# yanqinJiang/Animate3D

Measured on AMD Instinct MI355X. Metric: UNet denoise-steps/sec, 4view×16frame×512² MV-VDM @1/2/4/8 GPU, higher is better.
Workload: dtype bf16; 1 GPU; BASELINE config 2: 4 views x 16 frames x 512^2 px (64x64 latent), CFG-doubled batch V=8 videos, one MVUNetMotionModel.forward per step, SD1.5 MV-VDM UNet 1.53 B params, seeded synthetic weights; parallelism=single GPU

## Files before the change

### animate3d_amd/csrc/gemm_conv.hip

```cpp
#include "gemm_common.h"

namespace {

constexpr int BM = 128, BN = 128;
template <int BKT> struct TileCfg {
  static constexpr int LROW = BKT + 8;
  static constexpr int TILE_ELEMS = 128 * LROW;
  static constexpr int STAGE_BYTES = 2 * 2 * TILE_ELEMS * 2;
  static constexpr int EPI_BYTES = 4 * 32 * 68 * 4;
  static constexpr int SMEM_BYTES = STAGE_BYTES > EPI_BYTES ? STAGE_BYTES : EPI_BYTES;
  static constexpr int CPR = BKT / 8;
  static constexpr int RPT = 256 / CPR;
  static constexpr int NPASS = 128 / RPT;
};



template <int CONV, int EPI, int BKT, bool RES>
__global__ __launch_bounds__(256, (BKT == 64 ? 2 : 3)) void gemm_kernel(const GemmParams p) {
  using TC = TileCfg<BKT>;
  constexpr int LROW = TC::LROW, TILE_ELEMS = TC::TILE_ELEMS, NPASS = TC::NPASS, RPT = TC::RPT, BK = BKT;
  extern __shared__ __attribute__((aligned(16))) uint16_t smem[];
  const int tid = threadIdx.x;
  const int lane = tid & 63, wid = tid >> 6;
// ... 459 lines not shown
  p.X = (const uint16_t*)X; p.ldx = ldx; p.W = (const uint16_t*)W; p.ldw = ldw;
  p.bias = bias; p.rowbias = (const uint16_t*)rowbias; p.rb_div = rowbias ? rb_div : 1;
  p.R = (const uint16_t*)R; p.ldr = ldr; p.Y = (uint16_t*)Y; p.ldy = ldy;
  p.M = M; p.N = N; p.K = K; p.alpha = alpha; p.beta = beta;
  p.vec16 = (ldy % 8 == 0) && aligned16(Y) && (!R || (ldr % 8 == 0 && aligned16(R))) && (!rowbias || (N % 8 == 0 && aligned16(rowbias)));
  if (ws_needed) { *ws_needed = splitk_ws_bytes<0>(p, flags); return 0; }
  if (ws && ws_bytes > 0 && aligned16(ws)) { p.ws = (float*)ws; p.ws_bytes = ws_bytes; }
  return launch<0>((hipStream_t)stream, p, flags);
}

extern "C" int A3D_FN(a3d_gemm)(a3d_stream_t stream, const void* X, int64_t ldx, const void* W, int64_t ldw,
                             const float* bias, const void* rowbias, int64_t rb_div, const void* R, int64_t ldr,
                             void* Y, int64_t ldy, int64_t M, int64_t N, int64_t K, float alpha, float beta, int flags) {
  return gemm_entry(stream, X, ldx, W, ldw, bias, rowbias, rb_div, R, ldr, Y, ldy, M, N, K, alpha, beta, flags, nullptr, 0, nullptr);
}

extern "C" int A3D_FN(a3d_gemm_ws)(a3d_stream_t stream, const void* X, int64_t ldx, const void* W, int64_t ldw,
                                const float* bias, const void* rowbias, int64_t rb_div, const void* R, int64_t ldr,
                                void* Y, int64_t ldy, int64_t M, int64_t N, int64_t K, float alpha, float beta, int flags,
                                void* ws, int64_t ws_bytes, int64_t* ws_needed) {
  return gemm_entry(stream, X, ldx, W, ldw, bias, rowbias, rb_div, R, ldr, Y, ldy, M, N, K, alpha, beta, flags, ws, ws_bytes, ws_needed);
}

extern "C" int A3D_FN(a3d_gemm2)(a3d_stream_t stream, const void* X, int64_t ldx, const void* X2, int64_t ldx2, int64_t K1,
                              const void* W, int64_t ldw, const float* bias, void* Y, int64_t ldy, int64_t M, int64_t N, int64_t K, int flags) {
  if (!X || !X2 || !W || !Y || M <= 0 || N <= 0 || K <= 0 || K1 <= 0 || K1 >= K) return A3D_EINVAL;
  if (K % 64 != 0 || K1 % 64 != 0 || N % 8 != 0) return A3D_EINVAL;
  if (ldx % 8 != 0 || ldx2 % 8 != 0 || ldw % 8 != 0 || ldy % 8 != 0) return A3D_EINVAL;
  if (!aligned16(X) || !aligned16(X2) || !aligned16(W) || !aligned16(Y)) return A3D_EINVAL;
  if (bias && (reinterpret_cast<uintptr_t>(bias) & 15u)) return A3D_EINVAL;
  if (flags & ~(A3D_GEMM_RESERVED_CUS_MASK | A3D_GEMM_KERNEL_MASK)) return A3D_EINVAL;
  if (ldx2 % 64 != 0 || (uint64_t)ldx2 * 16u >= (1ull << 31)) return A3D_EUNSUPPORTED;
  GemmParams p{};
  p.X = (const uint16_t*)X; p.ldx = ldx; p.X2 = (const uint16_t*)X2; p.ldx2 = ldx2; p.K1 = K1;
  p.W = (const uint16_t*)W; p.ldw = ldw; p.bias = bias; p.rb_div = 1; p.Y = (uint16_t*)Y; p.ldy = ldy;
  p.M = M; p.N = N; p.K = K; p.alpha = 1.f; p.beta = 0.f; p.vec16 = 1;
  const int rc = try_launch_persist<0, EPI_LINEAR>((hipStream_t)stream, p, flags);
  return rc == -1000 ? A3D_EUNSUPPORTED : rc;
}

extern "C" int A3D_FN(a3d_gemm_f32out)(a3d_stream_t stream, const void* X, int64_t ldx, const void* W, int64_t ldw,
                                    const float* bias, float* Y, int64_t ldy, int64_t M, int64_t N, int64_t K, float alpha) {
  if (!X || !W || !Y || M <= 0 || N <= 0 || K <= 0) return A3D_EINVAL;
  if (K % 64 != 0 || N % 8 != 0 || ldx % 8 != 0 || ldw % 8 != 0 || ldy % 4 != 0) return A3D_EINVAL;
  if (!aligned16(X) || !aligned16(W) || !aligned16(Y)) return A3D_EINVAL;
  if (bias && (reinterpret_cast<uintptr_t>(bias) & 15u)) return A3D_EINVAL;
  GemmParams p{};
  p.X = (const uint16_t*)X; p.ldx = ldx; p.W = (const uint16_t*)W; p.ldw = ldw;
  p.bias = bias; p.rb_div = 1; p.Y = (uint16_t*)Y; p.ldy = ldy;
  p.M = M; p.N = N; p.K = K; p.alpha = alpha; p.beta = 0.f; p.vec16 = 1; p.out_f32 = 1;
  return launch<0>((hipStream_t)stream, p, 0);
}

static int conv_entry(a3d_stream_t stream, const void* X, const void* Wp, const float* bias,
                      const void* rowbias, int64_t rb_div, const void* R, void* Y,
                      int B, int H, int W, int Cin, int Cout, int stride, int up2x, int flags,
                      void* ws, int64_t ws_bytes, int64_t* ws_needed) {
  if (!X || !Wp || !Y || B <= 0 || H <= 0 || W <= 0) return A3D_EINVAL;
  if (Cin % 64 != 0 || Cout % 4 != 0 || (stride != 1 && stride != 2)) return A3D_EINVAL;
  if (up2x < 0 || up2x > 7 || (up2x > 1 && !(up2x & 1)) || (up2x && stride != 1)) return A3D_EINVAL;
  if (!aligned16(X) || !aligned16(Wp) || (reinterpret_cast<uintptr_t>(Y) & 7u)) return A3D_EINVAL;
// ... 43 lines not shown
```

### animate3d_amd/csrc/gemm_pp.hip

```cpp
#include "gemm_common.h"

namespace {

constexpr int PBM = 256;
template <int NB> struct PPCfg {
  static constexpr int BN = NB * 64;
  static constexpr int XBYTES = PBM * 128;
  static constexpr int WBYTES = BN * 128;
  static constexpr int EPI_BYTES = 8 * 32 * 68 * 4;
  static constexpr int STAGE = (XBYTES + WBYTES) > EPI_BYTES ? (XBYTES + WBYTES) : EPI_BYTES;
  static constexpr int BIAS_OFF = 2 * STAGE;
  static constexpr int BIAS_STRIDE = 2048;
  static constexpr int SMEM = 2 * STAGE + 2 * BIAS_STRIDE;
};

#ifndef A3D_PP_GM
#define A3D_PP_GM 8
#endif
constexpr int PP_GM = A3D_PP_GM;
A3D_DEV void pp_tile_coords(int64_t t, int64_t tiles_m, int64_t tiles_n, int64_t& tile_m, int64_t& tile_n) {
  const int64_t gsz = PP_GM * tiles_n;
  const int64_t blk = t / gsz;
  const int64_t first = blk * PP_GM;
  const int64_t gm = tiles_m - first < PP_GM ? tiles_m - first : PP_GM;
// ... 372 lines not shown
  static uint64_t attr_done = 0;
  if (int rc = a3d_once_per_device(attr_done, [] {
        return (int)hipFuncSetAttribute(reinterpret_cast<const void*>(&gemm_pp_kernel<CONV, EPI, NB, RES, SPLIT, TWO, DIRECT>),
                                        hipFuncAttributeMaxDynamicSharedMemorySize, PC::SMEM); })) return rc;
  const int64_t ntiles = p.tiles_m * p.tiles_n * (SPLIT ? p.ksplit : 1);
  const unsigned grid = (unsigned)(ntiles < cus ? ntiles : cus);
  gemm_pp_kernel<CONV, EPI, NB, RES, SPLIT, TWO, DIRECT><<<dim3(grid), dim3(512), PC::SMEM, stream>>>(p);
  if (int rc = a3d_launch_status()) return rc;
  if constexpr (SPLIT) {
    splitk_reduce_kernel<NB><<<dim3((unsigned)(p.tiles_m * p.tiles_n), NB), dim3(512), 0, stream>>>(p);
    return a3d_launch_status();
  }
  return 0;
}

template <int CONV>
int launch_pp_conv(int epi, int nb, hipStream_t stream, const GemmParams& p, int cus) {
  if (epi == EPI_GEGLU) {
    if constexpr (CONV == 0) { if (nb == 4) return launch_pp<0, EPI_GEGLU, 4, false>(stream, p, cus); }
    return A3D_EUNSUPPORTED;
  }
  if constexpr (CONV == 0) {
    if (p.X2 != nullptr) {
      if (p.R || p.ksplit > 1) return A3D_EUNSUPPORTED;
      if (nb == 5) return launch_pp<0, EPI_LINEAR, 5, false, false, true>(stream, p, cus);
      if (nb == 4) return launch_pp<0, EPI_LINEAR, 4, false, false, true>(stream, p, cus);
      return A3D_EUNSUPPORTED;
    }
  }
  if (p.ksplit > 1) {
    if (nb == 5) return launch_pp<CONV, EPI_LINEAR, 5, false, true>(stream, p, cus);
    if (nb == 4) return launch_pp<CONV, EPI_LINEAR, 4, false, true>(stream, p, cus);
    return A3D_EUNSUPPORTED;
  }
  if constexpr (CONV == 0) {
    if (p.direct) {
      if (nb == 5) return p.R ? launch_pp<0, EPI_LINEAR, 5, true, false, false, true>(stream, p, cus) : launch_pp<0, EPI_LINEAR, 5, false, false, false, true>(stream, p, cus);
      if (nb == 4) return p.R ? launch_pp<0, EPI_LINEAR, 4, true, false, false, true>(stream, p, cus) : launch_pp<0, EPI_LINEAR, 4, false, false, false, true>(stream, p, cus);
      return A3D_EUNSUPPORTED;
    }
  }
  if (nb == 5) return p.R ? launch_pp<CONV, EPI_LINEAR, 5, true>(stream, p, cus) : launch_pp<CONV, EPI_LINEAR, 5, false>(stream, p, cus);
  if (nb == 4) return p.R ? launch_pp<CONV, EPI_LINEAR, 4, true>(stream, p, cus) : launch_pp<CONV, EPI_LINEAR, 4, false>(stream, p, cus);
  return A3D_EUNSUPPORTED;
}

}

int A3D_FN(a3d_launch_gemm_pp)(int conv, int epi, int nb, hipStream_t stream, const GemmParams& p, int cus) {
// ... 5 lines not shown
```

### animate3d_amd/hip_ops.py

```python
from __future__ import annotations

import ctypes
import os
from dataclasses import dataclass
from typing import Optional

import torch

_LIB_PATH = os.path.join(os.path.dirname(os.path.abspath(__file__)), "lib", "libanimate3d_hip.so")
_lib = None

c_i64, c_int, c_f32, c_vp = ctypes.c_int64, ctypes.c_int, ctypes.c_float, ctypes.c_void_p


class _RowMapC(ctypes.Structure):
    _fields_ = [("gdiv", c_i64), ("ga", c_i64), ("gb", c_i64), ("seg_len", c_i64), ("seg_stride", c_i64), ("ld", c_i64)]


@dataclass(frozen=True)
class RowMap:
    gdiv: int
    ga: int
    gb: int
    seg_len: int
# ... 2 lines not shown
    def c(self, ld: int) -> _RowMapC:
        return _RowMapC(self.gdiv, self.ga, self.gb, self.seg_len, self.seg_stride, ld)


def rowmap_rows(m: RowMap, groups: int, step: int, length: int, device="cpu") -> torch.Tensor:
    g = torch.arange(0, groups, step, device=device).view(-1, 1)
    s = torch.arange(length, device=device).view(1, -1)
    return ((g // m.gdiv) * m.ga + (g % m.gdiv) * m.gb + (s // m.seg_len) * m.seg_stride + s % m.seg_len).reshape(-1)


def rowmap_covers(m: RowMap, groups: int, step: int, length: int, rows: int, device="cpu") -> bool:
    if (groups + step - 1) // step * length != rows:
        return False
    idx = rowmap_rows(m, groups, step, length, device)
    return bool(int(idx.min()) >= 0 and int(idx.max()) < rows and torch.unique(idx).numel() == rows)


_SIGNATURES = {
    "a3d_version": (ctypes.c_char_p, []),
    "a3d_gemm_bf16": (c_int, [c_vp, c_vp, c_i64, c_vp, c_i64, c_vp, c_vp, c_i64, c_vp, c_i64, c_vp, c_i64, c_i64, c_i64, c_i64, c_f32, c_f32, c_int]),
    "a3d_gemm_ws_bf16": (c_int, [c_vp, c_vp, c_i64, c_vp, c_i64, c_vp, c_vp, c_i64, c_vp, c_i64, c_vp, c_i64, c_i64, c_i64, c_i64, c_f32, c_f32, c_int,
                                 c_vp, c_i64, ctypes.POINTER(c_i64)]),
    "a3d_gemm2_bf16": (c_int, [c_vp, c_vp, c_i64, c_vp, c_i64, c_i64, c_vp, c_i64, c_vp, c_vp, c_i64, c_i64, c_i64, c_i64, c_int]),
    "a3d_gemm_geglu_bf16": (c_int, [c_vp, c_vp, c_i64, c_vp, c_i64, c_vp, c_vp, c_i64, c_i64, c_i64, c_i64, c_int]),
    "a3d_conv3x3_bf16": (c_int, [c_vp, c_vp, c_vp, c_vp, c_vp, c_i64, c_vp, c_vp, c_int, c_int, c_int, c_int, c_int, c_int, c_int, c_int]),
    "a3d_conv3x3_ws_bf16": (c_int, [c_vp, c_vp, c_vp, c_vp, c_vp, c_i64, c_vp, c_vp, c_int, c_int, c_int, c_int, c_int, c_int, c_int, c_int,
                                    c_vp, c_i64, ctypes.POINTER(c_i64)]),
    "a3d_flash_attn_bf16": (c_int, [c_vp, c_vp, c_vp, c_vp, c_vp, ctypes.POINTER(_RowMapC), ctypes.POINTER(_RowMapC), ctypes.POINTER(_RowMapC),
                                    c_int, c_int, c_int, c_i64, c_i64, c_f32, c_f32, c_int]),
    "a3d_flash_attn_counted_bf16": (c_int, [c_vp, c_vp, c_vp, c_vp, c_vp, ctypes.POINTER(_RowMapC), ctypes.POINTER(_RowMapC), ctypes.POINTER(_RowMapC),
                                            c_int, c_int, c_int, c_i64, c_i64, c_f32, c_f32, c_int, c_vp]),
    "a3d_flash_attn2_bf16": (c_int, [c_vp, c_vp, c_vp, c_vp, c_vp, c_vp, c_vp, ctypes.POINTER(_RowMapC), ctypes.POINTER(_RowMapC), ctypes.POINTER(_RowMapC),
                                     ctypes.POINTER(_RowMapC), c_int, c_int, c_int, c_i64, c_i64, c_i64, c_f32, c_f32, c_f32, c_int]),
    "a3d_temporal_attn_bf16": (c_int, [c_vp, c_vp, c_vp, c_vp, c_i64, c_vp, c_i64, c_int, c_int, c_i64, c_int, c_int, c_f32]),
    "a3d_temporal_attn_sharded_bf16": (c_int, [c_vp, c_vp, c_i64, c_vp, c_vp, c_i64, c_vp, c_i64, c_int, c_int, c_i64, c_int, c_int, c_f32,
                                               c_int, c_int, c_int, c_i64]),
    "a3d_group_norm_ws_floats": (c_i64, [c_int, c_i64, c_int]),
    "a3d_group_norm_bf16": (c_int, [c_vp, c_vp, c_vp, c_vp, c_vp, c_vp, c_int, c_i64, c_int, c_int, c_f32, c_int]),
    "a3d_group_norm2_bf16": (c_int, [c_vp, c_vp, c_int, c_vp, c_int, c_vp, c_vp, c_vp, c_vp, c_int, c_i64, c_int, c_f32, c_int]),
    "a3d_group_norm_sums_bf16": (c_int, [c_vp, c_vp, c_vp, c_vp, c_int, c_i64, c_int, c_int]),
    "a3d_group_norm_apply_bf16": (c_int, [c_vp, c_vp, c_vp, c_vp, c_vp, c_vp, c_int, c_i64, c_int, c_int, c_int]),
    "a3d_layer_norm_bf16": (c_int, [c_vp, c_vp, c_vp, c_vp, c_vp, c_vp, c_i64, c_int, c_f32, c_vp, c_i64, c_i64, c_vp, c_i64, c_i64]),
    "a3d_geglu_bf16": (c_int, [c_vp, c_vp, c_i64, c_vp, c_i64, c_i64, c_i64]),
    "a3d_silu_bf16": (c_int, [c_vp, c_vp, c_vp, c_i64]),
    "a3d_activation_bf16": (c_int, [c_vp, c_vp, c_vp, c_i64, c_int]),
    "a3d_concat_bf16": (c_int, [c_vp, c_vp, c_i64, c_vp, c_i64, c_vp, c_i64]),
# ... 174 lines not shown
        if rowbias is not None:
            self._act(rowbias, "gemm.rowbias")
            assert rowbias.is_contiguous() and rowbias.shape[1] == N
        if bias is not None:
            assert bias.dtype == torch.float32 and bias.numel() == N
        flags = self._gemm_flags(tile128, ring, direct)
        args = (self._stream(), _p(x), x.stride(0), _p(w), w.stride(0), _p(bias), _p(rowbias), rb_div,
                _p(residual), residual.stride(0) if residual is not None else 0, _p(y), y.stride(0), M, N, K, alpha, beta, flags)
        if self.split_k and self.split_k_gemm and not tile128 and M <= 32768 and K >= 1152:
            key = ("gemm", M, N, K, x.stride(0), w.stride(0), y.stride(0), rb_div if rowbias is not None else 0, flags)
            need = self._ws_plan.get(key)
            if need is None:
                q = c_i64(0)
                _check(self.lib.a3d_gemm_ws_bf16(*args, None, 0, ctypes.byref(q)), f"a3d_gemm_ws_bf16 (query) M={M} N={N} K={K}")
                need = self._ws_plan[key] = int(q.value)
            if need > 0:
                ws = self._workspace(need)
                _check(self.lib.a3d_gemm_ws_bf16(*args, _p(ws), need, None), f"a3d_gemm_ws_bf16 M={M} N={N} K={K}")
                return y
        rc = self.lib.a3d_gemm_bf16(*args)
        _check(rc, f"a3d_gemm_bf16 M={M} N={N} K={K}")
        return y

    def gemm2(self, xa, xb, w, bias=None):
        xa, xb, w = self._act(xa, "gemm2.xa"), self._act(xb, "gemm2.xb"), self._act(w, "gemm2.w")
        M, K1 = xa.shape
        K = K1 + xb.shape[1]
        N = w.shape[0]
        assert xb.shape[0] == M and w.shape[1] == K
        if K1 % 64 or K % 64 or N % 8:
            return None
        y = self.empty(M, N)
        rc = self.lib.a3d_gemm2_bf16(self._stream(), _p(xa), xa.stride(0), _p(xb), xb.stride(0), K1, _p(w), w.stride(0), _p(bias), _p(y), y.stride(0),
                                     M, N, K, self._gemm_flags(False))
        if rc == A3D_EUNSUPPORTED:
            return None
        _check(rc, f"a3d_gemm2_bf16 M={M} N={N} K={K1}+{K - K1}")
        return y

    @staticmethod
    def interleave_geglu(w: torch.Tensor) -> torch.Tensor:
        n = w.shape[0] // 2
        assert n % 32 == 0
        h, g = w[:n].reshape(n // 32, 32, *w.shape[1:]), w[n:].reshape(n // 32, 32, *w.shape[1:])
        return torch.stack([h, g], dim=1).reshape(w.shape).contiguous()

    def gemm_geglu(self, x, w_il, bias_il, *, tile128: bool = False):
        x, w_il = self._act(x, "geglu.x"), self._act(w_il, "geglu.w")
        M, K = x.shape
        N2 = w_il.shape[0]
        y = self.empty(M, N2 // 2)
        rc = self.lib.a3d_gemm_geglu_bf16(self._stream(), _p(x), x.stride(0), _p(w_il), w_il.stride(0), _p(bias_il), _p(y), y.stride(0), M, N2, K,
                                          self._gemm_flags(tile128))
        _check(rc, f"a3d_gemm_geglu_bf16 M={M} N2={N2} K={K}")
        return y

    def conv3x3(self, x, B: int, H: int, W: int, w, bias, *, stride: int = 1, up2x: bool = False, rowbias=None, rb_div: int = 1, residual=None,
                up_size=None, tile128: bool = False):
        x, w = self._act(x, "conv.x"), self._act(w, "conv.w")
        Cin = x.shape[1]
        Cout = w.shape[0]
# ... 440 lines not shown
```

### animate3d_amd/unet.py

```python
from __future__ import annotations

import math
import os
import re
from types import SimpleNamespace
from typing import Any, Dict, Optional, Tuple, Union

import torch
import torch.nn as nn

from . import modules as M
from .config import UNetConfig
from .embeddings import sine_pos_2d, sinusoidal_pos_1d
from .hip_ops import RowMap, on_model_device


class UNet3DConditionOutput:

    def __init__(self, sample: torch.Tensor):
        self.sample = sample

    def __getitem__(self, i):
        return (self.sample,)[i]

# ... 3 lines not shown
    if getattr(w, "_a3d_sink", None) is None:
        return w[r0:r1]
    from .autograd_ops import weight_rows
    return weight_rows(w, r0, r1)


class MVUNetMotionModel(nn.Module):
    def __init__(self, config: Optional[UNetConfig] = None, ops=None, num_views: Optional[int] = None,
                 device: Optional[Union[str, torch.device]] = None, **config_overrides):
        super().__init__()
        cfg = config if config is not None else UNetConfig(**config_overrides)
        self.config = cfg
        self.sample_size = cfg.sample_size
        self.num_views = num_views
        self._ops = ops
        self._ops_auto = False
        self._packed = None
        self._packed_frozen = None
        self._pack_grad = False
        self._train_ops = None
        self._active_ops = None
        self._cond = None
        self.stack_conditioning = True
        self._pe_cache: Dict[Tuple[int, int, int], torch.Tensor] = {}
        self.parallel = None
        self._frames = (0, 0)
        if len(cfg.block_out_channels) != len(cfg.down_has_attn):
            raise ValueError("block_out_channels and down_has_attn must have the same length")
        if 9 * cfg.in_channels > 64:
            raise ValueError(f"in_channels = {cfg.in_channels} is not supported (<= 7; the MV-VDM UNet has 4 — the 9-channel PIA conv_in "
                             "of unet_motion_mv_model.py:312-330 is not on this path)")
        ctx = torch.device(device) if device is not None else torch.device("cpu")
        with ctx:
            self._build(cfg)
            self._install_default_processors()

    def _build(self, cfg: UNetConfig):
        boc = cfg.block_out_channels
        temb_c = boc[0] * 4
        nlev = len(boc)
        self.conv_in = nn.Conv2d(cfg.in_channels, boc[0], 3, padding=1)
        self.time_embedding = M.TimestepEmbedding(boc[0], temb_c)
        if cfg.camera_embedding_dim is not None:
            self.camera_embedding = M.TimestepEmbedding(cfg.camera_embedding_dim, temb_c)
        self.encoder_hid_proj = None
        if cfg.encoder_hid_dim_type == "ip_image_proj":
# ... 296 lines not shown
    def _fold(self, a: torch.Tensor, b_t: torch.Tensor) -> torch.Tensor:
        ops = self._base_ops()
        dt = ops.act_dtype
        a, b_t = a.detach().float().contiguous(), b_t.detach().float().contiguous()
        ah, bh = a.to(dt), b_t.to(dt)
        al, bl = (a - ah.float()).to(dt), (b_t - bh.float()).to(dt)
        return ops.gemm_f32out(ah, bh) + ops.gemm_f32out(ah, bl) + ops.gemm_f32out(al, bh)

    def _pack_resnet(self, r: M.ResnetBlock2D):
        return SimpleNamespace(
            n1=(self._f(r.norm1.weight), self._f(r.norm1.bias)), eps=r.norm1.eps,
            c1=(self._conv_w(r.conv1), self._f(r.conv1.bias)),
            temb=(self._w(r.time_emb_proj.weight), self._f(r.time_emb_proj.bias)),
            n2=(self._f(r.norm2.weight), self._f(r.norm2.bias)),
            c2=(self._conv_w(r.conv2), self._f(r.conv2.bias)),
            sc=None if r.conv_shortcut is None else (self._conv_w(r.conv_shortcut), self._f(r.conv_shortcut.bias)))

    def _pack_ff(self, tb):
        return SimpleNamespace(n3=(self._f(tb.norm3.weight), self._f(tb.norm3.bias)),
                               ff1=(self._wcat([tb.ff.net[0].proj.weight], interleave=True),
                                    self._f(self.ops.interleave_geglu(self._d(tb.ff.net[0].proj.bias)))),
                               ff2=(self._w(tb.ff.net[2].weight), self._f(tb.ff.net[2].bias)))

    def _pack_t2d(self, t: M.Transformer2DModel):
        tb = t.transformer_blocks[0]
        a1, a2 = tb.attn1, tb.attn2
        p1, p2 = a1.processor, a2.processor
        if p1.kind not in ("mvdream", "mvdream_i2v") or p2.kind != "ip_adapter":
            raise TypeError("Transformer2D layers need a MVDream(I2V) processor on attn1 and an IPAdapter processor on attn2")
        qkv = [a1.to_k.weight, a1.to_v.weight, a1.to_q.weight]
        i2v = p1.kind == "mvdream_i2v"
        if i2v:
            qkv.append(p1.to_q_i2v.weight)
        out = SimpleNamespace(
            heads=a1.heads, i2v=i2v,
            norm=(self._f(t.norm.weight), self._f(t.norm.bias)),
            pin=(self._conv_w(t.proj_in), self._f(t.proj_in.bias)),
            n1=(self._f(tb.norm1.weight), self._f(tb.norm1.bias)),
            qkv=self._wcat(qkv),
            oi2v=(self._w(p1.to_out_i2v.weight), self._f(p1.to_out_i2v.bias)) if i2v else None,
            o1=(self._w(a1.to_out[0].weight), self._f(a1.to_out[0].bias)),
            n2=(self._f(tb.norm2.weight), self._f(tb.norm2.bias)),
            q2=self._w(a2.to_q.weight),
            kv_text=self._wcat([a2.to_k.weight, a2.to_v.weight]),
            kv_ip=[self._wcat([k.weight, v.weight]) for k, v in zip(p2.to_k_ip, p2.to_v_ip)],
            ip_scale=list(p2.scale), ip_tokens=list(p2.num_tokens),
            o2=(self._w(a2.to_out[0].weight), self._f(a2.to_out[0].bias)),
            pout=(self._conv_w(t.proj_out), self._f(t.proj_out.bias)))
        out.o1m = None
        if i2v and not self._pack_grad:
            wo, wi = a1.to_out[0].weight.detach().float(), p1.to_out_i2v.weight.detach().float()
            bias = a1.to_out[0].bias.detach().float()
            if p1.to_out_i2v.bias is not None:
                bias = bias + self._fold(p1.to_out_i2v.bias.detach().float()[None, :], wo)[0]
            out.o1m = (self._w(torch.cat([wo, self._fold(wo, wi.t())], dim=1)), self._f(bias))
        out.ff = self._pack_ff(tb)
        return out

    def _pack_motion(self, m: M.TransformerTemporalModel):
        tb = m.transformer_blocks[0]
        attns = []
        for a, ln in ((tb.attn1, tb.norm1), (tb.attn2, tb.norm2)):
            pr = a.processor
            if pr.kind != "spatio_temporal":
                raise TypeError("motion-module attention layers need a SpatioTemporalI2VAttnProcessor")
            C = a.to_q.weight.shape[0]
            if hasattr(pr, "time_pos_embed"):
                pe = pr.time_pos_embed.pe[0]
            else:
                pe = sinusoidal_pos_1d(C, self.config.motion_max_seq_length)[0].to(a.to_q.weight.device)
            proc_pe = hasattr(pr, "time_pos_embed")
            ct, cs, ci = pr.blend_coefficients_t() if self._pack_grad else pr.blend_coefficients()
            if self._pack_grad:
                self._coef_tensors.extend(c for c in (ct, cs, ci) if torch.is_tensor(c))
            ns = SimpleNamespace(
                heads=a.heads, spatial=pr.use_spatial_attn, image=pr.use_image_attn,
                spatial_pe=pr.use_spatial_attn and pr.use_spatial_encoding, camera_pe=pr.use_spatial_attn and pr.use_camera_encoding,
                n=(self._f(ln.weight), self._f(ln.bias)),
                qkv=self._wcat([a.to_q.weight, a.to_k.weight, a.to_v.weight]),
# ... 4 lines not shown
                ns.qkv_sp = self._wcat([pr.to_k_sp.weight, pr.to_v_sp.weight, pr.to_q_sp.weight])
                ns.osp = (self._w(pr.to_out_sp.weight), self._f(pr.to_out_sp.bias))
            if pr.use_image_attn:
                ns.qkv_img = self._wcat([pr.to_k_i2v.weight, pr.to_v_i2v.weight, pr.to_q_i2v.weight])
                ns.oimg = (self._w(pr.to_out_i2v.weight), self._f(pr.to_out_i2v.bias))
            ns.om = None
            if not self._pack_grad and (pr.use_spatial_attn or pr.use_image_attn):
                parts = [(ct, a.to_out[0])]
                if pr.use_spatial_attn:
                    parts.append((cs, pr.to_out_sp))
                if pr.use_image_attn:
                    parts.append((ci, pr.to_out_i2v))
                bias = None
                for c, lin in parts:
                    if lin.bias is not None:
                        bias = float(c) * lin.bias.detach().float() if bias is None else bias + float(c) * lin.bias.detach().float()
                ns.om = (self._w(torch.cat([float(c) * lin.weight.detach().float() for c, lin in parts], dim=1)), self._f(bias))
            attns.append(ns)
        out = SimpleNamespace(norm=(self._f(m.norm.weight), self._f(m.norm.bias)),
                              pin=(self._w(m.proj_in.weight), self._f(m.proj_in.bias)),
                              attns=attns,
                              pout=(self._w(m.proj_out.weight), self._f(m.proj_out.bias)))
        out.ff = self._pack_ff(tb)
        return out

    def _pack_block(self, blk: M.MotionBlock):
        return SimpleNamespace(
            resnets=[self._pack_resnet(r) for r in blk.resnets],
            t2d=[self._pack_t2d(t) for t in blk.attentions] if blk.has_cross_attention else None,
            motion=[self._pack_motion(m) for m in blk.motion_modules],
            down=None if blk.downsamplers is None else (self._conv_w(blk.downsamplers[0].conv), self._f(blk.downsamplers[0].conv.bias)),
            up=None if blk.upsamplers is None else (self._conv_w(blk.upsamplers[0].conv), self._f(blk.upsamplers[0].conv.bias)))

    def _pack(self):
        cfg = self.config
        dev = self.device
        te, P = self.time_embedding, SimpleNamespace()
        P.time = (self._w(te.linear_1.weight), self._f(te.linear_1.bias), self._w(te.linear_2.weight), self._f(te.linear_2.bias))
        P.cam = None
        if cfg.camera_embedding_dim is not None:
            ce = self.camera_embedding
            w1 = torch.zeros(ce.linear_1.weight.shape[0], 64, device=dev, dtype=torch.float32)
            w1[:, : cfg.camera_embedding_dim] = ce.linear_1.weight.detach().float()
            P.cam = (self._w(w1), self._f(ce.linear_1.bias), self._w(ce.linear_2.weight), self._f(ce.linear_2.bias))
        P.ip = None
        if self.encoder_hid_proj is not None:
# ... 102 lines not shown
        if isinstance(x, tuple):
            xa, xb = x
            sc = ops.gemm2(xa, xb, pk.sc[0], pk.sc[1]) if pk.sc is not None else None
            if sc is None:
                x = ops.concat(xa, xb)
                h = ops.group_norm(x, B2, L, pk.n1[0], pk.n1[1], g, pk.eps, True)
            else:
                h = ops.group_norm2(xa, xb, B2, L, pk.n1[0], pk.n1[1], g, pk.eps, True)
        else:
            h = ops.group_norm(x, B2, L, pk.n1[0], pk.n1[1], g, pk.eps, True)
        c = self._cond
        if c is not None and c.tp is not None and hasattr(pk, "temb_off"):
            o, N = pk.temb_off
            tp = c.tp[c.M * o: c.M * (o + N)].view(c.M, N)
        else:
            tp = ops.gemm(semb, pk.temb[0], pk.temb[1])
        h, _, _ = ops.conv3x3(h, B2, H, W, pk.c1[0], pk.c1[1], rowbias=tp, rb_div=rb_rows * L)
        h = ops.group_norm(h, B2, L, pk.n2[0], pk.n2[1], g, pk.eps, True)
        if sc is None:
            sc = x if pk.sc is None else ops.gemm(x, pk.sc[0], pk.sc[1])
        out, _, _ = ops.conv3x3(h, B2, H, W, pk.c2[0], pk.c2[1], residual=sc)
        return out

    def _ff(self, h, pk):
        ops = self.ops
        n3 = ops.layer_norm(h, pk.n3[0], pk.n3[1], 1e-5)
        u = ops.gemm_geglu(n3, pk.ff1[0], pk.ff1[1])
        return ops.gemm(u, pk.ff2[0], pk.ff2[1], residual=h)

    def _mv_maps(self, n, F, L):
        qm = RowMap(gdiv=F, ga=n * F * L, gb=L, seg_len=L, seg_stride=F * L)
        k0 = RowMap(gdiv=F, ga=n * F * L, gb=0, seg_len=L, seg_stride=F * L)
        return qm, k0

    def _mv_attention(self, x, w_kvq, C, V, n, F, L, heads, i2v, overlap=None, out_a=None, out_ai=None):
        ops, par = self.ops, self.parallel
        if par is not None and par.world == 1:
            par = None
        qm, k0 = self._mv_maps(n, F, L)
        b = V // n
        fsh = par is not None and par.frame_shards > 1
        vsh = par is not None and par.view_shards > 1
        N = n * par.view_shards if vsh else n

        def first_frame_kv():
            x0 = x.view(V, F, L, C)[:, 0].reshape(V * L, C) if par.frame_rank == 0 else None
            x0 = par.broadcast_frame0(x0, (V * L, C), x.dtype, x.device)
            if vsh:
                x0 = par.all_gather_views(x0, b)
            return ops.gemm(x0, _rows(w_kvq, 0, 2 * C)), RowMap(gdiv=F, ga=N * L, gb=0, seg_len=L, seg_stride=L)

# ... 23 lines not shown
            kv_all = par.all_gather_views_finish(pending, b)
        km, km0 = self._mv_maps(N, F, L)
        k, v = kv_all[:, :C], kv_all[:, C:]
        oa = {} if out_a is None else {"out": out_a}
        oi = {} if out_ai is None else {"out": out_ai}
        a = ops.flash_attn(qq[:, :C], k, v, qm, km, b * F, heads, n * L, N * L, **oa)
        ai = None
        if i2v and fsh:
            kv0, km0 = first_frame_kv()
            ai = ops.flash_attn(qq[:, C:2 * C], kv0[:, :C], kv0[:, C:], qm, km0, b * F, heads, n * L, N * L, **oi)
        elif i2v:
            ai = ops.flash_attn(qq[:, C:2 * C], k, v, qm, km0, b * F, heads, n * L, N * L, **oi)
        return a, ai, extra

    def _t2d(self, x, V, n, F, H, W, pk, text_rows, ip_rows, T):
        ops, g = self.ops, self.config.norm_num_groups
        B2, L, C = V * F, H * W, x.shape[1]
        h = ops.group_norm(x, B2, L, pk.norm[0], pk.norm[1], g, 1e-6, False)
        h = ops.gemm(h, pk.pin[0], pk.pin[1])
        n1 = ops.layer_norm(h, pk.n1[0], pk.n1[1], 1e-5)
        h = self._self_attention(n1, h, pk, V, n, F, L)
        n2 = ops.layer_norm(h, pk.n2[0], pk.n2[1], 1e-5)
        h = self._cross_attention(n2, h, pk, text_rows, ip_rows, T, B2, F, L)
        h = self._ff(h, pk.ff)
        return ops.gemm(h, pk.pout[0], pk.pout[1], residual=x)

    def _cross_attention(self, n2, residual, pk, text_rows, ip_rows, T, B2, F, L):
        ops = self.ops
        C = n2.shape[1]
        q2 = ops.gemm(n2, pk.q2)
        c = self._cond if hasattr(pk, "kv_off") else None
        kvt = c.kvt[:, pk.kv_off[0]: pk.kv_off[0] + 2 * C] if c is not None and c.kvt is not None else ops.gemm(text_rows, pk.kv_text)
        qc = RowMap(gdiv=1, ga=L, gb=0, seg_len=L, seg_stride=0)
        ca = None
        fused = getattr(ops, "flash_attn2", None)
        if fused is not None and len(ip_rows) == 1:
            kvi = c.kvi[:, pk.kv_off[0]: pk.kv_off[0] + 2 * C] if c is not None and c.kvi is not None else ops.gemm(ip_rows[0], pk.kv_ip[0])
            nt = pk.ip_tokens[0]
            ca = fused(q2, kvt[:, :C], kvt[:, C:], kvi[:, :C], kvi[:, C:], qc, RowMap(F, T, 0, T, 0), RowMap(F, nt, 0, nt, 0), B2, pk.heads,
                       L, T, nt, out_scale2=pk.ip_scale[0])
        if ca is None:
            ca = ops.flash_attn(q2, kvt[:, :C], kvt[:, C:], qc, RowMap(F, T, 0, T, 0), B2, pk.heads, L, T, accumulation_target=bool(ip_rows))
            for ipr, w, scale, nt in zip(ip_rows, pk.kv_ip, pk.ip_scale, pk.ip_tokens):
                kvi = ops.gemm(ipr, w)
                ops.flash_attn(q2, kvi[:, :C], kvi[:, C:], qc, RowMap(F, nt, 0, nt, 0), B2, pk.heads, L, nt,
                               out=ca, out_scale=scale, accumulate=True)
        return ops.gemm(ca, pk.o2[0], pk.o2[1], residual=residual)

# ... 68 lines not shown
            sums = par.all_reduce_frames(ops.group_norm_sums(x, V, F * L, g))
            cnt = float(F_all * L * (C // g))
            mean = sums[..., 0] / cnt
            var = (sums[..., 1] / cnt - mean * mean).clamp_min(0.0)
            stats = torch.stack([mean, 1.0 / torch.sqrt(var + 1e-6)], dim=-1).to(torch.float32).contiguous()
            h = ops.group_norm_apply(x, V, F * L, pk.norm[0], pk.norm[1], g, stats, False)
        else:
            h = ops.group_norm(x, V, F * L, pk.norm[0], pk.norm[1], g, 1e-6, False)
        h = ops.gemm(h, pk.pin[0], pk.pin[1])
        view0 = par.view_rank * n if par is not None else 0
        for a in pk.attns:
            pe_t = a.pe_t[f0:f0 + F]
            ln = lambda **kw: ops.layer_norm(h, a.n[0], a.n[1], 1e-5, **kw)
            if a.block_pe:
                nt = ns = nimg = ln(pe1=pe_t, pe1_div=L)
            else:
                if a.spatial_pe and not a.camera_pe and a.proc.spatial_encoding_type == "sinusoid":
                    pe_s, div_s = self._pe_spatial(C, H, W), 1
                else:
                    pe_s, div_s = self._pe_spatial_general(a, C, H, W, n, F, view0)
                nt, ns = ln(pe1=pe_t, pe1_div=L, pe2=pe_s, pe2_div=div_s, two=True)
                nimg = ln() if a.image else None
            h = self._motion_attn(h, nt, ns, nimg, a, V, n, F, L)
        h = self._ff(h, pk.ff)
        return ops.gemm(h, pk.pout[0], pk.pout[1], residual=x)

    def capture_graph(self, **inputs):
        clone = lambda v: v.clone() if torch.is_tensor(v) else ({k: w.clone() for k, w in v.items()} if isinstance(v, dict) else v)
        static = {k: clone(v) for k, v in inputs.items()}
        self(**static)
        side = torch.cuda.Stream(device=self.device)
        side.wait_stream(torch.cuda.current_stream(self.device))
        with torch.cuda.stream(side):
            self(**static)
        torch.cuda.current_stream(self.device).wait_stream(side)
        graph = torch.cuda.CUDAGraph()
        with torch.cuda.graph(graph):
            out = self(**static)

        def step(**new_inputs):
            for k, v in new_inputs.items():
                if torch.is_tensor(v):
                    static[k].copy_(v)
                elif isinstance(v, dict):
                    for kk, vv in v.items():
                        static[k][kk].copy_(vv)
                elif v != static[k]:
                    raise ValueError(f"capture_graph: non-tensor argument {k!r} is baked into the graph")
# ... 297 lines not shown
```

### include/animate3d_hip.h

```cpp
#ifndef ANIMATE3D_HIP_H
#define ANIMATE3D_HIP_H

#include <stdint.h>

#ifdef __cplusplus
extern "C" {
#endif

typedef void* a3d_stream_t;

enum {
  A3D_OK = 0,
  A3D_EINVAL = -1,
  A3D_EUNSUPPORTED = -2
};

enum { A3D_F32 = 0, A3D_BF16 = 1, A3D_F16 = 2 };

const char* a3d_version(void);

typedef struct a3d_rowmap {
  int64_t gdiv, ga, gb;
  int64_t seg_len, seg_stride;
  int64_t ld;
} a3d_rowmap;

#define A3D_GEMM_RESERVED_CUS_MASK 0xff
#define A3D_GEMM_KERNEL_MASK 0x300
#define A3D_GEMM_TILE128 0x100
#define A3D_GEMM_RING 0x200
#define A3D_GEMM_DIRECT 0x300
int a3d_gemm_bf16(a3d_stream_t stream, const void* X, int64_t ldx, const void* W, int64_t ldw,
                  const float* bias, const void* rowbias, int64_t rb_div, const void* R, int64_t ldr,
                  void* Y, int64_t ldy, int64_t M, int64_t N, int64_t K, float alpha, float beta, int flags);

int a3d_gemm_ws_bf16(a3d_stream_t stream, const void* X, int64_t ldx, const void* W, int64_t ldw,
                     const float* bias, const void* rowbias, int64_t rb_div, const void* R, int64_t ldr,
                     void* Y, int64_t ldy, int64_t M, int64_t N, int64_t K, float alpha, float beta, int flags,
                     void* ws, int64_t ws_bytes, int64_t* ws_needed);

int a3d_gemm2_bf16(a3d_stream_t stream, const void* X, int64_t ldx, const void* X2, int64_t ldx2, int64_t K1,
                   const void* W, int64_t ldw, const float* bias, void* Y, int64_t ldy, int64_t M, int64_t N, int64_t K, int flags);

int a3d_gemm_f32out_bf16(a3d_stream_t stream, const void* X, int64_t ldx, const void* W, int64_t ldw,
                         const float* bias, float* Y, int64_t ldy, int64_t M, int64_t N, int64_t K, float alpha);

int a3d_gemm_geglu_bf16(a3d_stream_t stream, const void* X, int64_t ldx, const void* W, int64_t ldw,
                        const float* bias, void* Y, int64_t ldy, int64_t M, int64_t N2, int64_t K, int flags);

int a3d_conv3x3_bf16(a3d_stream_t stream, const void* X, const void* Wp, const float* bias,
                     const void* rowbias, int64_t rb_div, const void* R, void* Y,
                     int B, int H, int W, int Cin, int Cout, int stride, int up2x, int flags);

int a3d_conv3x3_ws_bf16(a3d_stream_t stream, const void* X, const void* Wp, const float* bias,
                        const void* rowbias, int64_t rb_div, const void* R, void* Y,
                        int B, int H, int W, int Cin, int Cout, int stride, int up2x, int flags,
                        void* ws, int64_t ws_bytes, int64_t* ws_needed);

#define A3D_ATTN_ACCUMULATE 1
#define A3D_ATTN_CAUSAL 2
#define A3D_ATTN_EXACT 4
#define A3D_ATTN_PLAIN 8
int a3d_flash_attn_bf16(a3d_stream_t stream, const void* Q, const void* K, const void* V, void* O,
                        const a3d_rowmap* qmap, const a3d_rowmap* kmap, const a3d_rowmap* omap,
                        int groups, int heads, int head_dim, int64_t q_len, int64_t kv_len,
// ... 138 lines not shown

int a3d_dg_cells_f32(a3d_stream_t stream, int N, const float* xyz, const int64_t* plane_desc, int* cells);
int64_t a3d_dg_mean_partials(int N);
int a3d_dg_forward_f32(a3d_stream_t stream, int T, int N, int B, const float* xyz, const float* scaling, const float* rotation,
                       const float* timestamps, const float* grid, const int64_t* plane_desc, const float* weights, int flags,
                       const int* img_start, const int* img_list, float* sp, float* mpart, float* gmean, float* glob, float* means,
                       float* scales, float* rots);
int64_t a3d_dg_backward_ws_floats(int T, int N, const int64_t* plane_desc);
int a3d_dg_backward_f32(a3d_stream_t stream, int T, int N, int B, const float* xyz, const float* scaling, const float* rotation,
                        const float* timestamps, const float* grid, const int64_t* plane_desc, const float* weights, int flags,
                        const int* img_start, const int* img_list, const float* sp, const float* gmean, const float* glob,
                        const int* order, const int* starts, const float* d_means, const float* d_scales, const float* d_rots,
                        float* ws, float* d_grid, float* d_weights, float* d_scaling, float* d_rotation);

int a3d_gemm_f16(a3d_stream_t stream, const void* X, int64_t ldx, const void* W, int64_t ldw,
                  const float* bias, const void* rowbias, int64_t rb_div, const void* R, int64_t ldr,
                  void* Y, int64_t ldy, int64_t M, int64_t N, int64_t K, float alpha, float beta, int flags);
int a3d_gemm_ws_f16(a3d_stream_t stream, const void* X, int64_t ldx, const void* W, int64_t ldw,
                    const float* bias, const void* rowbias, int64_t rb_div, const void* R, int64_t ldr,
                    void* Y, int64_t ldy, int64_t M, int64_t N, int64_t K, float alpha, float beta, int flags,
                    void* ws, int64_t ws_bytes, int64_t* ws_needed);
int a3d_gemm2_f16(a3d_stream_t stream, const void* X, int64_t ldx, const void* X2, int64_t ldx2, int64_t K1,
                  const void* W, int64_t ldw, const float* bias, void* Y, int64_t ldy, int64_t M, int64_t N, int64_t K, int flags);
int a3d_gemm_f32out_f16(a3d_stream_t stream, const void* X, int64_t ldx, const void* W, int64_t ldw,
                         const float* bias, float* Y, int64_t ldy, int64_t M, int64_t N, int64_t K, float alpha);
int a3d_gemm_geglu_f16(a3d_stream_t stream, const void* X, int64_t ldx, const void* W, int64_t ldw,
                        const float* bias, void* Y, int64_t ldy, int64_t M, int64_t N2, int64_t K, int flags);
int a3d_conv3x3_f16(a3d_stream_t stream, const void* X, const void* Wp, const float* bias,
                     const void* rowbias, int64_t rb_div, const void* R, void* Y,
                     int B, int H, int W, int Cin, int Cout, int stride, int up2x, int flags);
int a3d_conv3x3_ws_f16(a3d_stream_t stream, const void* X, const void* Wp, const float* bias,
                       const void* rowbias, int64_t rb_div, const void* R, void* Y,
                       int B, int H, int W, int Cin, int Cout, int stride, int up2x, int flags,
                       void* ws, int64_t ws_bytes, int64_t* ws_needed);
int a3d_flash_attn_f16(a3d_stream_t stream, const void* Q, const void* K, const void* V, void* O,
                        const a3d_rowmap* qmap, const a3d_rowmap* kmap, const a3d_rowmap* omap,
                        int groups, int heads, int head_dim, int64_t q_len, int64_t kv_len,
                        float scale, float out_scale, int accumulate);
int a3d_flash_attn_counted_f16(a3d_stream_t stream, const void* Q, const void* K, const void* V, void* O,
                               const a3d_rowmap* qmap, const a3d_rowmap* kmap, const a3d_rowmap* omap,
                               int groups, int heads, int head_dim, int64_t q_len, int64_t kv_len,
                               float scale, float out_scale, int accumulate, unsigned int* counters);
int a3d_flash_attn2_f16(a3d_stream_t stream, const void* Q, const void* K, const void* V, const void* K2, const void* V2, void* O,
                        const a3d_rowmap* qmap, const a3d_rowmap* kmap, const a3d_rowmap* kmap2, const a3d_rowmap* omap,
                        int groups, int heads, int head_dim, int64_t q_len, int64_t kv_len, int64_t kv_len2,
                        float scale, float out_scale, float out_scale2, int accumulate);
// ... 65 lines not shown
```

Baseline: 2.386 denoise-steps/s.

## Fold FF output projection into transformer proj_out via dual-input residual GEMM

Result: no change. 2.402 denoise-steps/s (median of 6 runs) (+0.7%).

```diff
diff --git a/animate3d_amd/csrc/gemm_conv.hip b/animate3d_amd/csrc/gemm_conv.hip
--- a/animate3d_amd/csrc/gemm_conv.hip
+++ b/animate3d_amd/csrc/gemm_conv.hip
@@ -505,21 +505,34 @@
   return gemm_entry(stream, X, ldx, W, ldw, bias, rowbias, rb_div, R, ldr, Y, ldy, M, N, K, alpha, beta, flags, ws, ws_bytes, ws_needed);
 }
 
-extern "C" int A3D_FN(a3d_gemm2)(a3d_stream_t stream, const void* X, int64_t ldx, const void* X2, int64_t ldx2, int64_t K1,
-                              const void* W, int64_t ldw, const float* bias, void* Y, int64_t ldy, int64_t M, int64_t N, int64_t K, int flags) {
+static int gemm2_entry(a3d_stream_t stream, const void* X, int64_t ldx, const void* X2, int64_t ldx2, int64_t K1,
+                       const void* W, int64_t ldw, const float* bias, const void* R, int64_t ldr, void* Y, int64_t ldy,
+                       int64_t M, int64_t N, int64_t K, float alpha, float beta, int flags) {
   if (!X || !X2 || !W || !Y || M <= 0 || N <= 0 || K <= 0 || K1 <= 0 || K1 >= K) return A3D_EINVAL;
   if (K % 64 != 0 || K1 % 64 != 0 || N % 8 != 0) return A3D_EINVAL;
-  if (ldx % 8 != 0 || ldx2 % 8 != 0 || ldw % 8 != 0 || ldy % 8 != 0) return A3D_EINVAL;
-  if (!aligned16(X) || !aligned16(X2) || !aligned16(W) || !aligned16(Y)) return A3D_EINVAL;
+  if (ldx % 8 != 0 || ldx2 % 8 != 0 || ldw % 8 != 0 || ldy % 8 != 0 || (R && ldr % 8 != 0)) return A3D_EINVAL;
+  if (!aligned16(X) || !aligned16(X2) || !aligned16(W) || !aligned16(Y) || (R && !aligned16(R))) return A3D_EINVAL;
   if (bias && (reinterpret_cast<uintptr_t>(bias) & 15u)) return A3D_EINVAL;
   if (flags & ~(A3D_GEMM_RESERVED_CUS_MASK | A3D_GEMM_KERNEL_MASK)) return A3D_EINVAL;
   if (ldx2 % 64 != 0 || (uint64_t)ldx2 * 16u >= (1ull << 31)) return A3D_EUNSUPPORTED;
   GemmParams p{};
   p.X = (const uint16_t*)X; p.ldx = ldx; p.X2 = (const uint16_t*)X2; p.ldx2 = ldx2; p.K1 = K1;
-  p.W = (const uint16_t*)W; p.ldw = ldw; p.bias = bias; p.rb_div = 1; p.Y = (uint16_t*)Y; p.ldy = ldy;
-  p.M = M; p.N = N; p.K = K; p.alpha = 1.f; p.beta = 0.f; p.vec16 = 1;
+  p.W = (const uint16_t*)W; p.ldw = ldw; p.bias = bias; p.rb_div = 1; p.R = (const uint16_t*)R; p.ldr = ldr; p.Y = (uint16_t*)Y; p.ldy = ldy;
+  p.M = M; p.N = N; p.K = K; p.alpha = alpha; p.beta = beta; p.vec16 = 1;
   const int rc = try_launch_persist<0, EPI_LINEAR>((hipStream_t)stream, p, flags);
   return rc == -1000 ? A3D_EUNSUPPORTED : rc;
+}
+
+extern "C" int A3D_FN(a3d_gemm2)(a3d_stream_t stream, const void* X, int64_t ldx, const void* X2, int64_t ldx2, int64_t K1,
+                              const void* W, int64_t ldw, const float* bias, void* Y, int64_t ldy, int64_t M, int64_t N, int64_t K, int flags) {
+  return gemm2_entry(stream, X, ldx, X2, ldx2, K1, W, ldw, bias, nullptr, 0, Y, ldy, M, N, K, 1.f, 0.f, flags);
+}
+
+extern "C" int A3D_FN(a3d_gemm2_res)(a3d_stream_t stream, const void* X, int64_t ldx, const void* X2, int64_t ldx2, int64_t K1,
+                                  const void* W, int64_t ldw, const float* bias, void* Y, int64_t ldy, int64_t M, int64_t N, int64_t K, int flags,
+                                  const void* R, int64_t ldr, float alpha, float beta) {
+  if (!R) return A3D_EINVAL;
+  return gemm2_entry(stream, X, ldx, X2, ldx2, K1, W, ldw, bias, R, ldr, Y, ldy, M, N, K, alpha, beta, flags);
 }
 
 extern "C" int A3D_FN(a3d_gemm_f32out)(a3d_stream_t stream, const void* X, int64_t ldx, const void* W, int64_t ldw,
diff --git a/animate3d_amd/csrc/gemm_pp.hip b/animate3d_amd/csrc/gemm_pp.hip
--- a/animate3d_amd/csrc/gemm_pp.hip
+++ b/animate3d_amd/csrc/gemm_pp.hip
@@ -418,9 +418,9 @@
   }
   if constexpr (CONV == 0) {
     if (p.X2 != nullptr) {
-      if (p.R || p.ksplit > 1) return A3D_EUNSUPPORTED;
-      if (nb == 5) return launch_pp<0, EPI_LINEAR, 5, false, false, true>(stream, p, cus);
-      if (nb == 4) return launch_pp<0, EPI_LINEAR, 4, false, false, true>(stream, p, cus);
+      if (p.ksplit > 1) return A3D_EUNSUPPORTED;
+      if (nb == 5) return p.R ? launch_pp<0, EPI_LINEAR, 5, true, false, true>(stream, p, cus) : launch_pp<0, EPI_LINEAR, 5, false, false, true>(stream, p, cus);
+      if (nb == 4) return p.R ? launch_pp<0, EPI_LINEAR, 4, true, false, true>(stream, p, cus) : launch_pp<0, EPI_LINEAR, 4, false, false, true>(stream, p, cus);
       return A3D_EUNSUPPORTED;
     }
   }
diff --git a/animate3d_amd/hip_ops.py b/animate3d_amd/hip_ops.py
--- a/animate3d_amd/hip_ops.py
+++ b/animate3d_amd/hip_ops.py
@@ -48,6 +48,8 @@
     "a3d_gemm_ws_bf16": (c_int, [c_vp, c_vp, c_i64, c_vp, c_i64, c_vp, c_vp, c_i64, c_vp, c_i64, c_vp, c_i64, c_i64, c_i64, c_i64, c_f32, c_f32, c_int,
                                  c_vp, c_i64, ctypes.POINTER(c_i64)]),
     "a3d_gemm2_bf16": (c_int, [c_vp, c_vp, c_i64, c_vp, c_i64, c_i64, c_vp, c_i64, c_vp, c_vp, c_i64, c_i64, c_i64, c_i64, c_int]),
+    "a3d_gemm2_res_bf16": (c_int, [c_vp, c_vp, c_i64, c_vp, c_i64, c_i64, c_vp, c_i64, c_vp, c_vp, c_i64, c_i64, c_i64, c_i64, c_int,
+                                   c_vp, c_i64, c_f32, c_f32]),
     "a3d_gemm_geglu_bf16": (c_int, [c_vp, c_vp, c_i64, c_vp, c_i64, c_vp, c_vp, c_i64, c_i64, c_i64, c_i64, c_int]),
     "a3d_conv3x3_bf16": (c_int, [c_vp, c_vp, c_vp, c_vp, c_vp, c_i64, c_vp, c_vp, c_int, c_int, c_int, c_int, c_int, c_int, c_int, c_int]),
     "a3d_conv3x3_ws_bf16": (c_int, [c_vp, c_vp, c_vp, c_vp, c_vp, c_i64, c_vp, c_vp, c_int, c_int, c_int, c_int, c_int, c_int, c_int, c_int,
@@ -268,21 +270,39 @@
         _check(rc, f"a3d_gemm_bf16 M={M} N={N} K={K}")
         return y
 
-    def gemm2(self, xa, xb, w, bias=None):
+    has_gemm2_residual = True
+
+    def gemm2(self, xa, xb, w, bias=None, residual=None):
         xa, xb, w = self._act(xa, "gemm2.xa"), self._act(xb, "gemm2.xb"), self._act(w, "gemm2.w")
         M, K1 = xa.shape
         K = K1 + xb.shape[1]
         N = w.shape[0]
         assert xb.shape[0] == M and w.shape[1] == K
+        if bias is not None:
+            assert bias.dtype == torch.float32 and bias.numel() == N
         if K1 % 64 or K % 64 or N % 8:
             return None
         y = self.empty(M, N)
-        rc = self.lib.a3d_gemm2_bf16(self._stream(), _p(xa), xa.stride(0), _p(xb), xb.stride(0), K1, _p(w), w.stride(0), _p(bias), _p(y), y.stride(0),
-                                     M, N, K, self._gemm_flags(False))
+        args = (self._stream(), _p(xa), xa.stride(0), _p(xb), xb.stride(0), K1, _p(w), w.stride(0), _p(bias), _p(y), y.stride(0),
+                M, N, K, self._gemm_flags(False))
+        if residual is None:
+            name, rc = "a3d_gemm2_bf16", self.lib.a3d_gemm2_bf16(*args)
+        else:
+            self._act(residual, "gemm2.residual")
+            assert residual.shape == (M, N)
+            if residual.stride(0) % 8 or residual.data_ptr() % 16:
+                return None
+            name, rc = "a3d_gemm2_res_bf16", self.lib.a3d_gemm2_res_bf16(*args, _p(residual), residual.stride(0), 1.0, 1.0)
         if rc == A3D_EUNSUPPORTED:
             return None
-        _check(rc, f"a3d_gemm2_bf16 M={M} N={N} K={K1}+{K - K1}")
-        return y
+        _check(rc, f"{name} M={M} N={N} K={K1}+{K - K1}")
+        return y
+
+    def _persistent_takes(self, M: int, N: int, fill: float = 0.5) -> bool:
+        if M % 256:
+            return False
+        cus = torch.cuda.get_device_properties(self.device).multi_processor_count
+        return any(N % (64 * nb) == 0 and (M // 256) * (N // (64 * nb)) >= fill * cus for nb in (5, 4))
 
     @staticmethod
     def interleave_geglu(w: torch.Tensor) -> torch.Tensor:
diff --git a/animate3d_amd/unet.py b/animate3d_amd/unet.py
--- a/animate3d_amd/unet.py
+++ b/animate3d_amd/unet.py
@@ -49,6 +49,7 @@
         self._active_ops = None
         self._cond = None
         self.stack_conditioning = True
+        self._merge_ff_out = True
         self._pe_cache: Dict[Tuple[int, int, int], torch.Tensor] = {}
         self.parallel = None
         self._frames = (0, 0)
@@ -391,6 +392,16 @@
                                     self._f(self.ops.interleave_geglu(self._d(tb.ff.net[0].proj.bias)))),
                                ff2=(self._w(tb.ff.net[2].weight), self._f(tb.ff.net[2].bias)))
 
+    def _pack_ff_out(self, ff2: nn.Linear, pout):
+        if self._pack_grad or not getattr(self._base_ops(), "has_gemm2_residual", False):
+            return None
+        wp = pout.weight.detach().float().reshape(pout.weight.shape[0], -1)
+        w2 = ff2.weight.detach().float()
+        bias = pout.bias.detach().float() if pout.bias is not None else torch.zeros(wp.shape[0], device=wp.device)
+        if ff2.bias is not None:
+            bias = bias + self._fold(ff2.bias.detach().float()[None, :], wp)[0]
+        return (self._w(torch.cat([self._fold(wp, w2.t()), wp], dim=1)), self._f(bias))
+
     def _pack_t2d(self, t: M.Transformer2DModel):
         tb = t.transformer_blocks[0]
         a1, a2 = tb.attn1, tb.attn2
@@ -424,6 +435,7 @@
                 bias = bias + self._fold(p1.to_out_i2v.bias.detach().float()[None, :], wo)[0]
             out.o1m = (self._w(torch.cat([wo, self._fold(wo, wi.t())], dim=1)), self._f(bias))
         out.ff = self._pack_ff(tb)
+        out.ff.out = self._pack_ff_out(tb.ff.net[2], t.proj_out)
         return out
 
     def _pack_motion(self, m: M.TransformerTemporalModel):
@@ -474,6 +486,7 @@
                               attns=attns,
                               pout=(self._w(m.proj_out.weight), self._f(m.proj_out.bias)))
         out.ff = self._pack_ff(tb)
+        out.ff.out = self._pack_ff_out(tb.ff.net[2], m.proj_out) if len(m.transformer_blocks) == 1 else None
         return out
 
     def _pack_block(self, blk: M.MotionBlock):
@@ -622,11 +635,20 @@
         out, _, _ = ops.conv3x3(h, B2, H, W, pk.c2[0], pk.c2[1], residual=sc)
         return out
 
-    def _ff(self, h, pk):
+    def _ff(self, h, pk, pout, x):
         ops = self.ops
         n3 = ops.layer_norm(h, pk.n3[0], pk.n3[1], 1e-5)
         u = ops.gemm_geglu(n3, pk.ff1[0], pk.ff1[1])
-        return ops.gemm(u, pk.ff2[0], pk.ff2[1], residual=h)
+        if getattr(pk, "out", None) is not None and self._merge_ff_out and self._active_ops is None:
+            par = self.parallel if (self.parallel is not None and self.parallel.world > 1) else None
+            C = h.shape[1]
+            if C % 64 == 0 and ops._persistent_takes(h.shape[0] * (par.world if par is not None else 1), C, fill=1.0):
+                y = ops.gemm2(u, h, pk.out[0], pk.out[1], residual=x)
+                if y is None:
+                    y = ops.gemm(ops.concat(u, h), pk.out[0], pk.out[1], residual=x)
+                return y
+        h = ops.gemm(u, pk.ff2[0], pk.ff2[1], residual=h)
+        return ops.gemm(h, pout[0], pout[1], residual=x)
 
     def _mv_maps(self, n, F, L):
         qm = RowMap(gdiv=F, ga=n * F * L, gb=L, seg_len=L, seg_stride=F * L)
@@ -696,8 +718,7 @@
         h = self._self_attention(n1, h, pk, V, n, F, L)
         n2 = ops.layer_norm(h, pk.n2[0], pk.n2[1], 1e-5)
         h = self._cross_attention(n2, h, pk, text_rows, ip_rows, T, B2, F, L)
-        h = self._ff(h, pk.ff)
-        return ops.gemm(h, pk.pout[0], pk.pout[1], residual=x)
+        return self._ff(h, pk.ff, pk.pout, x)
 
     def _cross_attention(self, n2, residual, pk, text_rows, ip_rows, T, B2, F, L):
         ops = self.ops
@@ -812,8 +833,7 @@
                 nt, ns = ln(pe1=pe_t, pe1_div=L, pe2=pe_s, pe2_div=div_s, two=True)
                 nimg = ln() if a.image else None
             h = self._motion_attn(h, nt, ns, nimg, a, V, n, F, L)
-        h = self._ff(h, pk.ff)
-        return ops.gemm(h, pk.pout[0], pk.pout[1], residual=x)
+        return self._ff(h, pk.ff, pk.pout, x)
 
     def capture_graph(self, **inputs):
         clone = lambda v: v.clone() if torch.is_tensor(v) else ({k: w.clone() for k, w in v.items()} if isinstance(v, dict) else v)
diff --git a/include/animate3d_hip.h b/include/animate3d_hip.h
--- a/include/animate3d_hip.h
+++ b/include/animate3d_hip.h
@@ -41,6 +41,10 @@
 
 int a3d_gemm2_bf16(a3d_stream_t stream, const void* X, int64_t ldx, const void* X2, int64_t ldx2, int64_t K1,
                    const void* W, int64_t ldw, const float* bias, void* Y, int64_t ldy, int64_t M, int64_t N, int64_t K, int flags);
+
+int a3d_gemm2_res_bf16(a3d_stream_t stream, const void* X, int64_t ldx, const void* X2, int64_t ldx2, int64_t K1,
+                       const void* W, int64_t ldw, const float* bias, void* Y, int64_t ldy, int64_t M, int64_t N, int64_t K, int flags,
+                       const void* R, int64_t ldr, float alpha, float beta);
 
 int a3d_gemm_f32out_bf16(a3d_stream_t stream, const void* X, int64_t ldx, const void* W, int64_t ldw,
                          const float* bias, float* Y, int64_t ldy, int64_t M, int64_t N, int64_t K, float alpha);
@@ -225,6 +229,9 @@
                     void* ws, int64_t ws_bytes, int64_t* ws_needed);
 int a3d_gemm2_f16(a3d_stream_t stream, const void* X, int64_t ldx, const void* X2, int64_t ldx2, int64_t K1,
                   const void* W, int64_t ldw, const float* bias, void* Y, int64_t ldy, int64_t M, int64_t N, int64_t K, int flags);
+int a3d_gemm2_res_f16(a3d_stream_t stream, const void* X, int64_t ldx, const void* X2, int64_t ldx2, int64_t K1,
+                      const void* W, int64_t ldw, const float* bias, void* Y, int64_t ldy, int64_t M, int64_t N, int64_t K, int flags,
+                      const void* R, int64_t ldr, float alpha, float beta);
 int a3d_gemm_f32out_f16(a3d_stream_t stream, const void* X, int64_t ldx, const void* W, int64_t ldw,
                          const float* bias, float* Y, int64_t ldy, int64_t M, int64_t N, int64_t K, float alpha);
 int a3d_gemm_geglu_f16(a3d_stream_t stream, const void* X, int64_t ldx, const void* W, int64_t ldw,
```
